# zengxianyu/sketchedit

Measured on NVIDIA H100. Metric: images/sec 256x256 CelebA-HQ generator fwd, higher is better.
Workload: dtype bf16

## Files before the change

sketchedit_b200/csrc/se_conv_c8.cu:

```cuda
#include "se_conv_c8.h"

#include <stdlib.h>

#include <map>
#include <mutex>

#include "se_tc_device.cuh"

namespace se {

constexpr int C8_TH = 16, C8_TW = 8;
constexpr int C8_CONSUMER_WARPS = 8;
constexpr int C8_THREADS = 32 * C8_CONSUMER_WARPS + 32;
constexpr int C8_MAX_STAGES = 8;

__device__ __forceinline__ void ring_of(int i, int n, int shift, int& slot, uint32_t& phase) {
  if (shift >= 0) { slot = i & (n - 1); phase = (uint32_t)(i >> shift) & 1u; }
  else { const int qd = i / n; slot = i - qd * n; phase = (uint32_t)qd & 1u; }
}

template <int NT, bool kF16, int R64, int M64, int R32>
__global__ void __launch_bounds__(C8_THREADS, 1)
conv_c8_kernel(const __grid_constant__ CUtensorMap tmA, const C8Params p) {
  extern __shared__ __align__(1024) uint8_t smem_raw[];
  uint8_t* smem = reinterpret_cast<uint8_t*>((reinterpret_cast<uintptr_t>(smem_raw) + 1023) & ~uintptr_t(1023));
  const bool halo = (p.mode == C8_HALO);
  constexpr int b64_bytes = NT * 128, b32_bytes = NT * 64;
  constexpr int b_bytes = R64 * b64_bytes + R32 * b32_bytes;
  const int stage_a = halo ? 0 : p.a_bytes;
  const int stage_b = p.resident ? 0 : b_bytes;
  const int stage_bytes = stage_a + stage_b;
  const bool staged = stage_bytes > 0;
  uint8_t* sHalo = smem;
  uint8_t* sWres = sHalo + (halo ? p.a_bufs * p.a_bytes : 0);
  uint8_t* sStages = sWres + (p.resident ? p.wres_bytes : 0);
  uint8_t* tail = sStages + (size_t)p.num_stages * stage_bytes;
  uint64_t* full_bar = reinterpret_cast<uint64_t*>(tail);
  uint64_t* empty_bar = full_bar + C8_MAX_STAGES;
  uint64_t* a_full = empty_bar + C8_MAX_STAGES;
  uint64_t* a_empty = a_full + C8_MAX_ABUFS;
  uint64_t* wres_bar = a_empty + C8_MAX_ABUFS;
  float* bias_s = reinterpret_cast<float*>(wres_bar + 2);

  const int warp = threadIdx.x >> 5;
  const int lane = threadIdx.x & 31;
  const bool clustered = p.cluster > 1;
  const uint32_t rank = clustered ? cluster_ctarank() : 0u;
  if (threadIdx.x == 0) {
    for (int i = 0; i < C8_MAX_STAGES; ++i) {
      mbar_init(&full_bar[i], 1);
      mbar_init(&empty_bar[i], C8_CONSUMER_WARPS * p.cluster);
    }
    for (int i = 0; i < C8_MAX_ABUFS; ++i) {
      mbar_init(&a_full[i], 1);
      mbar_init(&a_empty[i], C8_CONSUMER_WARPS);
    }
    mbar_init(wres_bar, 1);
    asm volatile("fence.mbarrier_init.release.cluster;" ::: "memory");
  }
  const int cst_n = NT + 32;
  epi_fill_constants(bias_s, cst_n, p.bias, p.e, threadIdx.x, C8_THREADS);
  if (clustered) cluster_sync();
  else __syncthreads();

  const int total_tiles = p.N * p.tiles_x * p.tiles_y;
  const int ksteps = p.ksteps;
  const int first_tile = (int)blockIdx.x - (int)rank;

  if (warp == C8_CONSUMER_WARPS) {
    if (lane == 0) asm volatile("prefetch.tensormap [%0];" ::"l"(reinterpret_cast<uint64_t>(&tmA)) : "memory");
    if (p.resident && elect_one()) {
      mbar_expect_tx(wres_bar, (uint32_t)p.wres_bytes);
      for (int off = 0; off < p.wres_bytes; off += 65536) {
        const int n = min(65536, p.wres_bytes - off);
        bulk_load_1d(sWres + off, p.w + off, (uint32_t)n, wres_bar);
      }
    }
    __syncwarp();
    const int b_split = (b_bytes >> 11) << 10;
    const int b_off = rank ? b_split : 0, b_len = clustered ? (rank ? b_bytes - b_split : b_split) : b_bytes;
    int stage = 0, iter = 0;
    uint32_t phase = 0;
    int tx = blockIdx.x % p.tiles_x, ty = (blockIdx.x / p.tiles_x) % p.tiles_y, img = blockIdx.x / (p.tiles_x * p.tiles_y);
    for (int tile = blockIdx.x; tile - (int)rank < total_tiles; tile += gridDim.x, ++iter) {
      if (tile != (int)blockIdx.x) {
        tx += p.step_x;
        if (tx >= p.tiles_x) { tx -= p.tiles_x; ++ty; }
        ty += p.step_y;
        if (ty >= p.tiles_y) { ty -= p.tiles_y; ++img; }
        img += p.step_img;
      }
      const int x0 = tx * C8_TW, y0 = ty * C8_TH;
      const bool load_a = tile < total_tiles;
      if (halo && load_a) {
        int ab;
        uint32_t aphase;
        ring_of(iter, p.a_bufs, p.a_shift, ab, aphase);
        mbar_wait(&a_empty[ab], aphase ^ 1, 5);
        if (elect_one()) {
          mbar_expect_tx(&a_full[ab], (uint32_t)p.a_tx_bytes);
          tma_load_4d(sHalo + (size_t)ab * p.a_bytes, &tmA, &a_full[ab], (x0 - p.pad_x0) * 8, y0 - p.pad_y0, p.x_cb_off, img);
        }
        __syncwarp();
      }
      if (staged) {
        for (int ks = 0; ks < ksteps; ++ks) {
          mbar_wait(&empty_bar[stage], phase ^ 1, 1);
          uint8_t* st = sStages + (size_t)stage * stage_bytes;
          if (elect_one()) {
            mbar_expect_tx(&full_bar[stage], (uint32_t)((halo || !load_a ? 0 : p.a_tx_bytes) + stage_b));
            if (!p.resident) {
              const uint8_t* src = p.w + (size_t)ks * b_bytes + b_off;
              if (clustered) bulk_load_1d_multicast(st + stage_a + b_off, src, (uint32_t)b_len, &full_bar[stage], 0x3);
              else bulk_load_1d(st + stage_a, src, (uint32_t)b_len, &full_bar[stage]);
            }
            if (!halo && load_a) {
              const int t = ks / p.cpt, ch = ks - t * p.cpt;
              tma_load_4d(st, &tmA, &full_bar[stage], (x0 + p.dx[t]) * 8, y0 + p.dy[t], p.x_cb_off + p.tap_cb[t] + 8 * ch, img);
            }
          }
          __syncwarp();
          if (++stage == p.num_stages) { stage = 0; phase ^= 1; }
        }
      }
    }
  } else {
    const int wg = warp >> 2, wq = warp & 3;
    const uint32_t smem_base = smem_u32(smem);
    const uint32_t off_wres = halo ? (uint32_t)(p.a_bufs * p.a_bytes) : 0u;
    const uint32_t off_stages = off_wres + (p.resident ? (uint32_t)p.wres_bytes : 0u);
    const uint32_t a_m = (uint32_t)wg * 8u * (uint32_t)p.sbo_bytes;
    const uint32_t n_u64 = p.ntaps * p.n64;
    const int ncls = p.ncls;
    const uint32_t tpi = (uint32_t)(p.tiles_x * p.tiles_y);
    const uint32_t cst_s = smem_u32(bias_s);
    const bool elu = p.e.epi == EPI_GATE_ELU, paired = p.e.paired != 0;
    if (p.resident) mbar_wait(wres_bar, 0, 6);
    auto release = [&](uint64_t* bar) {
      __syncwarp();
      if (lane == 0) mbar_arrive(bar);
    };
    auto release_stage = [&](int s) {
      __syncwarp();
      if (lane == 0) {
        mbar_arrive(&empty_bar[s]);
        if (clustered) mbar_arrive_cluster(&empty_bar[s], rank ^ 1u);
      }
    };
    float acc[NT / 2];
#pragma unroll
    for (int i = 0; i < NT / 2; ++i) acc[i] = 0.0f;
    int stage = 0;
    uint32_t phase = 0;
    const int my_tiles = (first_tile < total_tiles) ? (total_tiles - first_tile + (int)gridDim.x - 1) / (int)gridDim.x : 0;
    const int nv = my_tiles * ncls;
    const bool pingpong = p.resident && ksteps == 1;
    for (int v = 0; v < nv; ++v) {
      const int riter = ncls == 1 ? v : v / ncls, cls = v - riter * ncls;
      const int tile = (int)blockIdx.x + riter * (int)gridDim.x;
      if (tile >= total_tiles) {
        for (int ks = 0; ks < ksteps; ++ks) {
          mbar_wait(&full_bar[stage], phase, 3);
          release_stage(stage);
          if (++stage == p.num_stages) { stage = 0; phase ^= 1; }
        }
        continue;
      }
      const uint32_t img_u = (uint32_t)tile / tpi, rem = (uint32_t)tile - img_u * tpi;
      const uint32_t ty_u = rem / (uint32_t)p.tiles_x;
      const int img = (int)img_u, ty = (int)ty_u, tx = (int)(rem - ty_u * (uint32_t)p.tiles_x);
      int ab = 0;
      if (halo) {
        uint32_t aph;
        ring_of(riter, p.a_bufs, p.a_shift, ab, aph);
        mbar_wait(&a_full[ab], aph, 7);
      }
      if (pingpong && (wg == 1 || v > 0)) named_bar_sync(wg == 0 ? 2 : 1, 256);
      int prev = -1;
      for (int ks = 0; ks < ksteps; ++ks) {
        if (staged) mbar_wait(&full_bar[stage], phase, 3);
        const uint32_t st = smem_base + off_stages + (uint32_t)stage * stage_bytes;
        const uint32_t sB = p.resident ? smem_base + off_wres + (uint32_t)cls * (uint32_t)p.cls_bytes + (uint32_t)ks * b_bytes : st + stage_a;
        const uint32_t sA = (halo ? smem_base + (uint32_t)ab * p.a_bytes : st) + a_m;
        const int ub = cls * C8_CLS_UNITS;
        const int u0 = ub + ks * R64, v0 = ub + (int)n_u64 + ks * R32;
        const uint32_t acc0 = ks ? 1u : 0u;
        wg_fence();
        wg_fence_acc(acc);
#pragma unroll
        for (int j = 0; j < R64; ++j) {
          const uint32_t a0 = sA + p.aoff[u0 + j];
          const uint32_t b0 = sB + (uint32_t)(j * b64_bytes);
#pragma unroll
          for (int k = 0; k < M64; ++k)
            Wgmma<NT, kF16, 0>::mma(acc, wg_desc(a0 + k * p.kstep_bytes, p.lbo_bytes, p.sbo_bytes, WG_SW_NONE),
                                    wg_desc(b0 + 32u * k, 16u, 1024u, WG_SW128), j + k ? 1u : acc0);
        }
#pragma unroll
        for (int j = 0; j < R32; ++j) {
          const uint32_t a0 = sA + p.aoff[v0 + j];
          const uint32_t b0 = sB + (uint32_t)(R64 * b64_bytes + j * b32_bytes);
#pragma unroll
          for (int k = 0; k < 2; ++k)
            Wgmma<NT, kF16, 0>::mma(acc, wg_desc(a0 + k * p.kstep_bytes, p.lbo_bytes, p.sbo_bytes, WG_SW_NONE),
                                    wg_desc(b0 + 32u * k, 16u, 512u, WG_SW64), R64 + j + k ? 1u : acc0);
        }
        wg_commit();
        if (staged) {
          if (prev >= 0) {
            wg_wait<1>();
            release_stage(prev);
          }
          prev = stage;
          if (++stage == p.num_stages) { stage = 0; phase ^= 1; }
        }
      }
      if (pingpong && (wg == 0 || v + 1 < nv)) named_bar_arrive(wg == 0 ? 1 : 2, 256);
      wg_wait<0>();
      wg_fence_acc(acc);
      if (prev >= 0) release_stage(prev);
      if (halo && cls == ncls - 1) release(&a_empty[ab]);
      const int ooy = ncls > 1 ? p.cls_ooy[cls] : p.e.ooy, oox = ncls > 1 ? p.cls_oox[cls] : p.e.oox;
      size_t base[2];
      bool ok[2];
#pragma unroll
      for (int h = 0; h < 2; ++h) {
        const int ry = 8 * wg + 2 * wq + h, rx = lane >> 2;
        const int py = ty * C8_TH + ry, px = tx * C8_TW + rx;
        ok[h] = py < p.Ho && px < p.Wo;
        base[h] = epi_pixel_offset(p.e, img, py * p.e.osy + ooy, px * p.e.osx + oox, 2 * (lane & 3));
      }
      if (elu) {
        if (kF16 || paired) conv_epilogue<NT, kF16, true, true>(p.e, cst_s, acc, base, ok, lane);
        else conv_epilogue<NT, false, true, false>(p.e, cst_s, acc, base, ok, lane);
      } else {
        if (kF16 || paired) conv_epilogue<NT, kF16, false, true>(p.e, cst_s, acc, base, ok, lane);
        else conv_epilogue<NT, false, false, false>(p.e, cst_s, acc, base, ok, lane);
      }
    }
  }
  if (clustered) cluster_sync();
}

void fill_epi(const ConvParams& c, int NT, EpiParams* e) {
  e->y = c.y; e->out_c8 = c.out_c8;
  e->Hout = c.Hout; e->Wout = c.Wout; e->ldo = c.ldo; e->choff = c.choff;
  e->osy = c.osy; e->ooy = c.ooy; e->osx = c.osx; e->oox = c.oox;
  e->epi = c.epi; e->scale = c.scale;
  e->Cout = c.Cout; e->NT = NT;
  e->blk_split = c.out_blk_split > 0 ? c.out_blk_split : (1 << 20);
  e->blk_jump = c.out_blk_split > 0 ? c.out_blk_jump : 0;
  e->par_stride = c.out_par_stride > 0 ? c.out_par_stride : (c.ldo >> 2);
  const long long plane = c.out_c8 == 2 ? (long long)(c.Hout / 2) * (c.Wout / 2) : (long long)c.Hout * c.Wout;
  e->blk_stride = (int)(c.out_c8 ? plane * 8 : 8);
  e->goff = gated_goff(c.Cout);
  e->paired = (c.out_c8 != 0 || (((c.ldo | c.choff) & 1) == 0 && c.Cout / 2 == e->goff)) ? 1 : 0;
  e->split_stride = (int)c.out_split_stride;
}
typedef CUresult (*EncodeTiledFn)(CUtensorMap*, CUtensorMapDataType, cuuint32_t, void*, const cuuint64_t*, const cuuint64_t*,
                                  const cuuint32_t*, const cuuint32_t*, CUtensorMapInterleave, CUtensorMapSwizzle,
                                  CUtensorMapL2promotion, CUtensorMapFloatOOBfill);
static EncodeTiledFn c8_encode_fn() {
  static EncodeTiledFn fn = nullptr;
  if (!fn) {
    void* p = nullptr;
    cudaDriverEntryPointQueryResult qres;
    if (cudaGetDriverEntryPoint("cuTensorMapEncodeTiled", &p, cudaEnableDefault, &qres) != cudaSuccess || qres != cudaDriverEntryPointSuccess || !p) return nullptr;
    fn = reinterpret_cast<EncodeTiledFn>(p);
  }
  return fn;
// ... 36 lines not shown
  L->mode = (halo_bytes <= 72 * 1024) ? C8_HALO : C8_PERTAP;
  if (L->mode == C8_HALO) {
    L->HR = HR; L->WR = WR; L->pad_y0 = -mn_y; L->pad_x0 = -mn_x;
  } else {
    L->HR = C8_TH; L->WR = C8_TW; L->pad_y0 = 0; L->pad_x0 = 0;
    L->cb_in = (w.n64 * 64 + w.n32 * 32) / 8;
  }
  L->a_tx_bytes = L->cb_in * L->HR * L->WR * 16;
  L->a_bytes = (L->a_tx_bytes + 1023) / 1024 * 1024;
  L->resident = (wbytes <= kResidentMax) && (2 * L->a_bytes + wbytes <= kSmemBudget);
  if (L->resident && L->mode == C8_HALO) {
    w.r64 = ntaps * w.n64;
    w.r32 = ntaps * w.n32;
  } else if (L->mode == C8_PERTAP || (w.n64 > 0 && w.n32 > 0)) { w.r64 = w.n64; w.r32 = w.n32; }
  else {
    const int unit = w.n64 ? w.NT * 128 : w.NT * 64, total = ntaps * (w.n64 ? w.n64 : w.n32);
    int best = 1;
    for (int k = 1; k <= 8 && k <= total; ++k)
      if (total % k == 0 && k * unit <= 48 * 1024) best = k;
    if (w.n64) { w.r64 = best; w.r32 = 0; } else { w.r64 = 0; w.r32 = best; }
  }
  if (L->mode == C8_PERTAP && w.n32 == 0 && w.n64 > 1 && 2 * (L->a_bytes + w.NT * w.n64 * 128) > kSmemBudget) {
    L->chunks_per_tap = w.n64;
    L->cb_in = 8;
    L->a_tx_bytes = L->cb_in * L->HR * L->WR * 16;
    L->a_bytes = (L->a_tx_bytes + 1023) / 1024 * 1024;
    w.r64 = 1;
  }
  if (L->mode == C8_PERTAP) SE_REQUIRE(tc_ksteps(w) == ntaps * L->chunks_per_tap, "per-tap stages must be whole taps or whole chunks");
  return 0;
}

typedef void (*C8Kernel)(CUtensorMap, C8Params);
struct C8Inst { int nt; bool f16; int r64, m64, r32; C8Kernel fn; };
#define C8_INST(nt, f16, r64, m64, r32) {nt, f16, r64, m64, r32, conv_c8_kernel<nt, f16, r64, m64, r32>}
static const C8Inst kC8Insts[] = {
    C8_INST(32, false, 0, 0, 9),
    C8_INST(48, false, 0, 0, 9),
    C8_INST(48, false, 4, 3, 0),
    C8_INST(48, false, 5, 3, 0),
    C8_INST(96, false, 0, 0, 9),
    C8_INST(96, false, 4, 4, 4),
    C8_INST(96, false, 5, 3, 0),
    C8_INST(96, false, 9, 3, 0),
    C8_INST(96, false, 3, 3, 0),
    C8_INST(192, false, 1, 3, 0),
    C8_INST(192, false, 1, 4, 0),
    C8_INST(192, false, 1, 4, 1),
    C8_INST(32, true, 0, 0, 27),
    C8_INST(48, true, 0, 0, 3),
    C8_INST(48, true, 12, 3, 0),
    C8_INST(48, true, 15, 3, 0),
    C8_INST(96, true, 0, 0, 3),
    C8_INST(96, true, 1, 3, 0),
    C8_INST(96, true, 1, 4, 1),
    C8_INST(96, true, 3, 3, 0),
    C8_INST(192, true, 1, 3, 0),
    C8_INST(192, true, 1, 4, 0),
    C8_INST(192, true, 1, 4, 1),
};
#undef C8_INST
static C8Kernel c8_kernel(const C8Layer& L, bool f16) {
  const TcWeights& w = L.w;
  const int r64 = w.n64 ? w.r64 : 0, r32 = w.n32 ? w.r32 : 0, m64 = r64 ? L.mmas64 : 0;
  for (const C8Inst& k : kC8Insts)
    if (k.nt == w.NT && k.f16 == f16 && k.r64 == r64 && k.m64 == m64 && k.r32 == r32) return k.fn;
  return nullptr;
}
static int c8_set_smem_attr(int bytes) {
  for (const C8Inst& k : kC8Insts) SE_CUDA_OK(cudaFuncSetAttribute(k.fn, cudaFuncAttributeMaxDynamicSharedMemorySize, bytes));
  return 0;
}
int c8_instantiated(const C8Layer& L, bool f16, const std::string& name) {
  const TcWeights& w = L.w;
  SE_REQUIRE(c8_kernel(L, f16) != nullptr,
             "layer " + name + (f16 ? " (split-half)" : "") + ": no conv_c8_kernel instantiation for N = " + std::to_string(w.NT) +
                 ", k-step of " + std::to_string(w.n64 ? w.r64 : 0) + " x " + std::to_string(L.mmas64) + " + " +
                 std::to_string(w.n32 ? w.r32 : 0) + " x 2 MMAs (se_conv_c8.cu: kC8Insts)");
  return 0;
}
static void c8_launch_config(cudaLaunchConfig_t* cfg, cudaLaunchAttribute* attr, int grid, int smem_bytes, int cluster, cudaStream_t stream) {
  *cfg = cudaLaunchConfig_t();
  cfg->gridDim = dim3(grid);
  cfg->blockDim = dim3(C8_THREADS);
  cfg->dynamicSmemBytes = smem_bytes;
  cfg->stream = stream;
  if (cluster > 1) {
    attr->id = cudaLaunchAttributeClusterDimension;
    attr->val.clusterDim.x = cluster;
    attr->val.clusterDim.y = 1;
    attr->val.clusterDim.z = 1;
    cfg->attrs = attr;
    cfg->numAttrs = 1;
  }
}
static int c8_max_clusters(C8Kernel k, int smem_bytes, int* out) {
  static std::mutex mu;
  static std::map<std::pair<C8Kernel, int>, int> cache;
  std::lock_guard<std::mutex> lock(mu);
  auto it = cache.find({k, smem_bytes});
  if (it == cache.end()) {
    cudaLaunchConfig_t cfg;
    cudaLaunchAttribute attr;
    c8_launch_config(&cfg, &attr, 2 * g_sms, smem_bytes, 2, 0);
    int n = 0;
    SE_CUDA_OK(cudaOccupancyMaxActiveClusters(&n, k, &cfg));
    SE_REQUIRE(n > 0, "no 2-CTA cluster of conv_c8_kernel fits on the device");
    it = cache.emplace(std::make_pair(k, smem_bytes), n).first;
  }
  *out = it->second;
  return 0;
}

static const int kGroupSmemMax = 222 * 1024;

int c8_configure_group(C8Group* G, int ncls, int ntaps, const int8_t (*dy)[8], const int8_t (*dx)[8], const int* ooy, const int* oox, int Ci, int Cout) {
  if (ncls < 2 || ncls > C8_MAX_CLS || ntaps > 8) return 1;
  int mn_y = 0, mx_y = 0, mn_x = 0, mx_x = 0;
  for (int c = 0; c < ncls; ++c)
    for (int t = 0; t < ntaps; ++t) {
      mn_y = dy[c][t] < mn_y ? dy[c][t] : mn_y; mx_y = dy[c][t] > mx_y ? dy[c][t] : mx_y;
      mn_x = dx[c][t] < mn_x ? dx[c][t] : mn_x; mx_x = dx[c][t] > mx_x ? dx[c][t] : mx_x;
    }
  C8Layer& L = G->geo;
  L = C8Layer();
  TcWeights& w = L.w;
  w.ntaps = ntaps;
  w.n64 = Ci / 64;
  int rem = Ci - 64 * w.n64;
  if (rem > 32) { ++w.n64; rem = 0; }
  w.n32 = rem > 0 ? 1 : 0;
  w.NT = (gated_goff(Cout) + Cout / 2 + 15) / 16 * 16;
  w.n_tiles = 1;
  w.img_bytes = 0;
  w.r64 = ntaps * w.n64;
  w.r32 = ntaps * w.n32;
  L.mmas64 = Ci == 48 ? 3 : 4;
// ... 51 lines not shown
  p.cls_bytes = grp ? grp->cls_bytes : 0;
  for (int k = 0; k < C8_MAX_CLS; ++k) { p.cls_ooy[k] = grp && k < grp->ncls ? grp->ooy[k] : 0; p.cls_oox[k] = grp && k < grp->ncls ? grp->oox[k] : 0; }
  if (L.stem) { p.lbo_bytes = 16; p.kstep_bytes = 32; }
  else { p.lbo_bytes = L.HR * L.WR * 16; p.kstep_bytes = 2 * p.lbo_bytes; }
  p.sbo_bytes = L.WR * 16;
  p.bias = c.bias;
  fill_epi(c, w.NT, &p.e);
  {
    const bool halo = (L.mode == C8_HALO);
    const int n_u64 = c.ntaps * w.n64, n_u32 = c.ntaps * w.n32;
    SE_REQUIRE(n_u64 + n_u32 < C8_MAX_UNITS, "too many K units");
    SE_REQUIRE(!grp || n_u64 + n_u32 <= C8_CLS_UNITS, "too many K units per class");
    for (int k = 0; k < (grp ? grp->ncls : 1); ++k)
      for (int u = 0; u < n_u64 + n_u32; ++u) {
        const bool is64 = u < n_u64;
        const int t = is64 ? u / w.n64 : u - n_u64;
        const int cb0 = L.chunks_per_tap > 1 ? 0 : (halo ? L.tap_cb[t] : 0) + (is64 ? (u - t * w.n64) * 8 : w.n64 * 8);
        const int tdy = grp ? grp->dy[k][t] : c.dy[t], tdx = grp ? grp->dx[k][t] : c.dx[t];
        const int oy = halo ? tdy + L.pad_y0 : 0, ox = halo ? tdx + L.pad_x0 : 0;
        p.aoff[k * C8_CLS_UNITS + u] = (uint32_t)((cb0 * L.HR + oy) * L.WR + ox) * 16u;
      }
  }
  SE_REQUIRE(c.Cout % 2 == 0 && (c.out_dt == DT_BF16 || c.out_dt == DT_F16X2), "gated epilogue needs even Cout, 16-bit out");
  SE_REQUIRE(!c.out_c8 || c.choff % 8 == 0, "C8 output needs a channel offset multiple of 8");
  SE_REQUIRE(!c.f16x2 || c.out_c8 != 0, "split-half output is channel-blocked");
  SE_REQUIRE(c.out_c8 != 2 || (c.Hout % 2 == 0 && c.Wout % 2 == 0 && c.ldo % 4 == 0 && (c.Cout / 2) % 8 == 0),
             "space-to-depth output: even size, whole channel blocks");
  {
    const long long plane = c.out_c8 == 2 ? (long long)(c.Hout / 2) * (c.Wout / 2) : (long long)c.Hout * c.Wout;
    SE_REQUIRE((long long)(w.NT / 16) * (c.out_c8 ? 8 * plane : 8) + 8LL * p.e.blk_jump < (1LL << 31), "output block offsets must fit in 31 bits");
  }

  const int total_tiles = p.N * p.tiles_x * p.tiles_y;
  const int smem_budget = grp ? kGroupSmemMax - 4096 : kSmemBudget;
  const int b_bytes = tc_stage_b_bytes(w);
  const int stage_bytes = (L.mode == C8_HALO ? 0 : L.a_bytes) + (L.resident ? 0 : b_bytes);
  int fixed = (L.resident ? p.wres_bytes : 0);
  p.a_bufs = 2;
  if (L.mode == C8_HALO) {
    if (fixed + 2 * L.a_bytes + 3 * stage_bytes > smem_budget) p.a_bufs = 1;
    if (stage_bytes == 0)
      while (p.a_bufs < C8_MAX_ABUFS && fixed + 2 * p.a_bufs * L.a_bytes <= smem_budget) p.a_bufs *= 2;
    fixed += p.a_bufs * L.a_bytes;
  }
  p.a_shift = -1;
  for (int sh = 0; sh < 4; ++sh) if ((1 << sh) == p.a_bufs) p.a_shift = sh;
  SE_REQUIRE(p.a_bufs <= C8_MAX_ABUFS, "halo ring plan");
  SE_REQUIRE(!grp || (p.a_bufs >= 2 && p.ksteps == 1), "fused classes need two halo buffers and a single k-step");
  SE_REQUIRE(!(L.resident && p.ksteps == 1) || p.a_bufs >= 2, "ping-pong warpgroups need two halo buffers");
  int stages = stage_bytes ? (smem_budget - fixed) / stage_bytes : 1;
  if (stages > C8_MAX_STAGES) stages = C8_MAX_STAGES;
  SE_REQUIRE(stages >= (stage_bytes ? 2 : 1), "shared memory plan does not fit");
  p.num_stages = stages;
  const int smem_bytes = 1024 + fixed + stages * stage_bytes + (2 * C8_MAX_STAGES + 2 * C8_MAX_ABUFS + 2) * 8 + 3 * (p.NT + 32) * 4 + 64;

  EncodeTiledFn enc = c8_encode_fn();
  SE_REQUIRE(enc != nullptr, "cuTensorMapEncodeTiled not available from the driver");
  if (!g_sms) {
    int dev = 0;
    SE_CUDA_OK(cudaGetDevice(&dev));
    SE_CUDA_OK(cudaDeviceGetAttribute(&g_sms, cudaDevAttrMultiProcessorCount, dev));
    SE_CUDA_OK(cudaDeviceGetAttribute(&g_optin, cudaDevAttrMaxSharedMemoryPerBlockOptin, dev));
    { int rc_attr = c8_set_smem_attr(g_optin); if (rc_attr) return rc_attr; }
  }
  SE_REQUIRE(smem_bytes <= g_optin, "shared memory plan exceeds the opt-in limit");

  CUtensorMap tmA;
  {
    cuuint64_t dims[4] = {(cuuint64_t)c.Wi * 8, (cuuint64_t)c.Hi, (cuuint64_t)c.ldx, (cuuint64_t)c.N};
    cuuint64_t strides[3] = {(cuuint64_t)c.Wi * 16, (cuuint64_t)c.Hi * c.Wi * 16, (cuuint64_t)c.ldx * c.Hi * c.Wi * 16};
    cuuint32_t box[4] = {(cuuint32_t)(L.WR * 8), (cuuint32_t)L.HR, (cuuint32_t)L.cb_in, 1};
    cuuint32_t estr[4] = {1, 1, 1, 1};
    CUresult r = enc(&tmA, CU_TENSOR_MAP_DATA_TYPE_BFLOAT16, 4, const_cast<void*>(c.x), dims, strides, box, estr,
                     CU_TENSOR_MAP_INTERLEAVE_NONE, CU_TENSOR_MAP_SWIZZLE_NONE, CU_TENSOR_MAP_L2_PROMOTION_L2_256B,
                     CU_TENSOR_MAP_FLOAT_OOB_FILL_NONE);
    SE_REQUIRE(r == CUDA_SUCCESS, "cuTensorMapEncodeTiled(C8) failed, CUresult=" + std::to_string((int)r));
  }
  const C8Kernel kernel = c8_kernel(L, p.f16 != 0);
  SE_REQUIRE(kernel != nullptr, "no conv_c8_kernel instantiation for the layer's plan (N = " + std::to_string(p.NT) + ")");
  p.cluster = L.resident ? 1 : 2;
  int grid = total_tiles < g_sms ? total_tiles : g_sms;
  if (p.cluster > 1) {
    int max_clusters = 0;
    { int rc_occ = c8_max_clusters(kernel, smem_bytes, &max_clusters); if (rc_occ) return rc_occ; }
    const int pairs = (total_tiles + 1) / 2;
    grid = 2 * (pairs < max_clusters ? pairs : max_clusters);
  }
  p.step_x = grid % p.tiles_x;
  p.step_y = (grid / p.tiles_x) % p.tiles_y;
  p.step_img = grid / (p.tiles_x * p.tiles_y);
  cudaLaunchConfig_t cfg;
  cudaLaunchAttribute attr;
  c8_launch_config(&cfg, &attr, grid, smem_bytes, p.cluster, stream);
  SE_CUDA_OK(cudaLaunchKernelEx(&cfg, kernel, tmA, p));
  return 0;
}

}
```

sketchedit_b200/csrc/se_tc_device.cuh:

```cuda
#pragma once
#include <cuda_fp16.h>

#include "se_common.cuh"
#include "se_wgmma.cuh"

namespace se {

__device__ __forceinline__ uint32_t smem_u32(const void* p) { return (uint32_t)__cvta_generic_to_shared(p); }

__device__ __forceinline__ void mbar_init(uint64_t* bar, uint32_t count) {
  asm volatile("mbarrier.init.shared::cta.b64 [%0], %1;" ::"r"(smem_u32(bar)), "r"(count));
}
__device__ __forceinline__ void mbar_expect_tx(uint64_t* bar, uint32_t bytes) {
  asm volatile("mbarrier.arrive.expect_tx.shared::cta.b64 _, [%0], %1;" ::"r"(smem_u32(bar)), "r"(bytes) : "memory");
}
__device__ __forceinline__ void mbar_arrive(uint64_t* bar) {
  asm volatile("mbarrier.arrive.shared::cta.b64 _, [%0];" ::"r"(smem_u32(bar)) : "memory");
}
__device__ __forceinline__ void mbar_wait(uint64_t* bar, uint32_t parity, int tag) {
  (void)tag;
  asm volatile(
      "{\n\t.reg .pred p;\n\t.reg .b64 t0, t1;\n\t.reg .b32 n;\n\t"
      "mov.u64 t0, 0;\n\t"
      "OUTER_%=:\n\t"
// ... 32 lines not shown
               : "memory");
}

__device__ __forceinline__ uint32_t cluster_ctarank() {
  uint32_t r;
  asm volatile("mov.u32 %0, %%cluster_ctarank;" : "=r"(r));
  return r;
}
__device__ __forceinline__ void cluster_sync() {
  asm volatile("barrier.cluster.arrive.release;\n\tbarrier.cluster.wait.acquire;" ::: "memory");
}
__device__ __forceinline__ void mbar_arrive_cluster(uint64_t* bar, uint32_t cta) {
  asm volatile("{\n\t.reg .b32 ra;\n\tmapa.shared::cluster.u32 ra, %0, %1;\n\tmbarrier.arrive.release.cta.shared::cluster.b64 _, [ra];\n\t}"
               ::"r"(smem_u32(bar)), "r"(cta) : "memory");
}

__device__ __forceinline__ bool elect_one() {
  uint32_t pred;
  asm volatile("{\n\t.reg .pred p;\n\telect.sync _|p, 0xffffffff;\n\tselp.u32 %0, 1, 0, p;\n\t}" : "=r"(pred));
  return pred != 0;
}

enum : uint32_t { WG_SW_NONE = 0, WG_SW128 = 1, WG_SW64 = 2 };
__device__ __forceinline__ uint64_t wg_desc(uint32_t smem_addr, uint32_t lbo_bytes, uint32_t sbo_bytes, uint32_t layout) {
  return (uint64_t)((smem_addr & 0x3FFFF) >> 4) | ((uint64_t)((lbo_bytes >> 4) & 0x3FFF) << 16) |
         ((uint64_t)((sbo_bytes >> 4) & 0x3FFF) << 32) | ((uint64_t)layout << 62);
}
__device__ __forceinline__ void wg_fence() { asm volatile("wgmma.fence.sync.aligned;" ::: "memory"); }
__device__ __forceinline__ void wg_commit() { asm volatile("wgmma.commit_group.sync.aligned;" ::: "memory"); }
template <int N>
__device__ __forceinline__ void wg_wait() { asm volatile("wgmma.wait_group.sync.aligned %0;" ::"n"(N) : "memory"); }
__device__ __forceinline__ void named_bar_sync(int id, int n) { asm volatile("bar.sync %0, %1;" ::"r"(id), "r"(n) : "memory"); }
__device__ __forceinline__ void named_bar_arrive(int id, int n) { asm volatile("bar.arrive %0, %1;" ::"r"(id), "r"(n) : "memory"); }
template <int R>
__device__ __forceinline__ void wg_fence_acc(float (&d)[R]) {
#pragma unroll
  for (int i = 0; i < R; ++i) asm volatile("" : "+f"(d[i])::"memory");
}
__device__ __forceinline__ int frag_row(int w, int lane, int h) { return 16 * w + (lane >> 2) + 8 * h; }
__device__ __forceinline__ int frag_col(int lane, int j) { return 8 * j + 2 * (lane & 3); }

__device__ __forceinline__ float tanh_approx(float x) {
  float y;
  asm("tanh.approx.f32 %0, %1;" : "=f"(y) : "f"(x));
  return y;
}
__device__ __forceinline__ float ex2_approx(float x) {
  float y;
  asm("ex2.approx.ftz.f32 %0, %1;" : "=f"(y) : "f"(x));
  return y;
}
__device__ __forceinline__ float rcp_approx(float x) {
  float y;
  asm("rcp.approx.ftz.f32 %0, %1;" : "=f"(y) : "f"(x));
  return y;
}
__device__ __forceinline__ uint32_t pack_f16x2(float lo, float hi) {
  __half2 v = __floats2half2_rn(lo, hi);
  return *reinterpret_cast<uint32_t*>(&v);
}

__device__ __forceinline__ void epi_fill_constants(float* cst, int n, const float* bias, const EpiParams& e, int tid, int nthreads) {
  const int half = e.Cout >> 1;
  for (int i = tid; i < n; i += nthreads) {
    const int ch = i < half ? i : (i >= e.goff && i < e.goff + half ? half + i - e.goff : -1);
    const float b = (bias != nullptr && ch >= 0 && ch < e.Cout) ? bias[ch] : 0.0f;
// ... 104 lines not shown
```

Baseline: 4725.

## Add ping-pong consumer warpgroups with full-tile accumulators for streamed-weight convs

Adds a ping-pong variant of the implicit-GEMM conv kernel. Each consumer warpgroup now owns a whole 16-row tile with two accumulator sets and alternates tiles with the other warpgroup through named barriers, so one group's epilogue overlaps the other's WGMMA mainloop. The variant adds a full producer warpgroup and uses setmaxnreg to move registers to the consumers. It is selected for non-resident, non-f16 layers with at least two tiles per SM, and it raises the shared-memory budget for those layers. The cost is higher register pressure, fewer pipeline stages per stage reader, and a more complex launch path.

```diff
diff --git a/sketchedit_b200/csrc/se_conv_c8.cu b/sketchedit_b200/csrc/se_conv_c8.cu
--- a/sketchedit_b200/csrc/se_conv_c8.cu
+++ b/sketchedit_b200/csrc/se_conv_c8.cu
@@ -12,6 +12,8 @@
 constexpr int C8_TH = 16, C8_TW = 8;
 constexpr int C8_CONSUMER_WARPS = 8;
 constexpr int C8_THREADS = 32 * C8_CONSUMER_WARPS + 32;
+constexpr int C8_PP_THREADS = 32 * C8_CONSUMER_WARPS + 128;
+constexpr int C8_PP_PRODUCER_REGS = 40, C8_PP_CONSUMER_REGS = 232;
 constexpr int C8_MAX_STAGES = 8;
 
 __device__ __forceinline__ void ring_of(int i, int n, int shift, int& slot, uint32_t& phase) {
@@ -19,9 +21,11 @@
   else { const int qd = i / n; slot = i - qd * n; phase = (uint32_t)qd & 1u; }
 }
 
-template <int NT, bool kF16, int R64, int M64, int R32>
-__global__ void __launch_bounds__(C8_THREADS, 1)
+template <int NT, bool kF16, int R64, int M64, int R32, bool kPP>
+__global__ void __launch_bounds__(kPP ? C8_PP_THREADS : C8_THREADS, 1)
 conv_c8_kernel(const __grid_constant__ CUtensorMap tmA, const C8Params p) {
+  constexpr int kThreads = kPP ? C8_PP_THREADS : C8_THREADS;
+  constexpr int kStageReaders = kPP ? 4 : C8_CONSUMER_WARPS;
   extern __shared__ __align__(1024) uint8_t smem_raw[];
   uint8_t* smem = reinterpret_cast<uint8_t*>((reinterpret_cast<uintptr_t>(smem_raw) + 1023) & ~uintptr_t(1023));
   const bool halo = (p.mode == C8_HALO);
@@ -49,17 +53,17 @@
   if (threadIdx.x == 0) {
     for (int i = 0; i < C8_MAX_STAGES; ++i) {
       mbar_init(&full_bar[i], 1);
-      mbar_init(&empty_bar[i], C8_CONSUMER_WARPS * p.cluster);
+      mbar_init(&empty_bar[i], kStageReaders * p.cluster);
     }
     for (int i = 0; i < C8_MAX_ABUFS; ++i) {
       mbar_init(&a_full[i], 1);
-      mbar_init(&a_empty[i], C8_CONSUMER_WARPS);
+      mbar_init(&a_empty[i], kStageReaders);
     }
     mbar_init(wres_bar, 1);
     asm volatile("fence.mbarrier_init.release.cluster;" ::: "memory");
   }
   const int cst_n = NT + 32;
-  epi_fill_constants(bias_s, cst_n, p.bias, p.e, threadIdx.x, C8_THREADS);
+  epi_fill_constants(bias_s, cst_n, p.bias, p.e, threadIdx.x, kThreads);
   if (clustered) cluster_sync();
   else __syncthreads();
 
@@ -67,69 +71,72 @@
   const int ksteps = p.ksteps;
   const int first_tile = (int)blockIdx.x - (int)rank;
 
-  if (warp == C8_CONSUMER_WARPS) {
-    if (lane == 0) asm volatile("prefetch.tensormap [%0];" ::"l"(reinterpret_cast<uint64_t>(&tmA)) : "memory");
-    if (p.resident && elect_one()) {
-      mbar_expect_tx(wres_bar, (uint32_t)p.wres_bytes);
-      for (int off = 0; off < p.wres_bytes; off += 65536) {
-        const int n = min(65536, p.wres_bytes - off);
-        bulk_load_1d(sWres + off, p.w + off, (uint32_t)n, wres_bar);
-      }
-    }
-    __syncwarp();
-    const int b_split = (b_bytes >> 11) << 10;
-    const int b_off = rank ? b_split : 0, b_len = clustered ? (rank ? b_bytes - b_split : b_split) : b_bytes;
-    int stage = 0, iter = 0;
-    uint32_t phase = 0;
-    int tx = blockIdx.x % p.tiles_x, ty = (blockIdx.x / p.tiles_x) % p.tiles_y, img = blockIdx.x / (p.tiles_x * p.tiles_y);
-    for (int tile = blockIdx.x; tile - (int)rank < total_tiles; tile += gridDim.x, ++iter) {
-      if (tile != (int)blockIdx.x) {
-        tx += p.step_x;
-        if (tx >= p.tiles_x) { tx -= p.tiles_x; ++ty; }
-        ty += p.step_y;
-        if (ty >= p.tiles_y) { ty -= p.tiles_y; ++img; }
-        img += p.step_img;
-      }
-      const int x0 = tx * C8_TW, y0 = ty * C8_TH;
-      const bool load_a = tile < total_tiles;
-      if (halo && load_a) {
-        int ab;
-        uint32_t aphase;
-        ring_of(iter, p.a_bufs, p.a_shift, ab, aphase);
-        mbar_wait(&a_empty[ab], aphase ^ 1, 5);
-        if (elect_one()) {
-          mbar_expect_tx(&a_full[ab], (uint32_t)p.a_tx_bytes);
-          tma_load_4d(sHalo + (size_t)ab * p.a_bytes, &tmA, &a_full[ab], (x0 - p.pad_x0) * 8, y0 - p.pad_y0, p.x_cb_off, img);
-        }
-        __syncwarp();
-      }
-      if (staged) {
-        for (int ks = 0; ks < ksteps; ++ks) {
-          mbar_wait(&empty_bar[stage], phase ^ 1, 1);
-          uint8_t* st = sStages + (size_t)stage * stage_bytes;
+  if (warp >= C8_CONSUMER_WARPS) {
+    if constexpr (kPP) setmaxnreg_dec<C8_PP_PRODUCER_REGS>();
+    if (warp == C8_CONSUMER_WARPS) {
+      if (lane == 0) asm volatile("prefetch.tensormap [%0];" ::"l"(reinterpret_cast<uint64_t>(&tmA)) : "memory");
+      if (p.resident && elect_one()) {
+        mbar_expect_tx(wres_bar, (uint32_t)p.wres_bytes);
+        for (int off = 0; off < p.wres_bytes; off += 65536) {
+          const int n = min(65536, p.wres_bytes - off);
+          bulk_load_1d(sWres + off, p.w + off, (uint32_t)n, wres_bar);
+        }
+      }
+      __syncwarp();
+      const int b_split = (b_bytes >> 11) << 10;
+      const int b_off = rank ? b_split : 0, b_len = clustered ? (rank ? b_bytes - b_split : b_split) : b_bytes;
+      int stage = 0, iter = 0;
+      uint32_t phase = 0;
+      int tx = blockIdx.x % p.tiles_x, ty = (blockIdx.x / p.tiles_x) % p.tiles_y, img = blockIdx.x / (p.tiles_x * p.tiles_y);
+      for (int tile = blockIdx.x; tile - (int)rank < total_tiles; tile += gridDim.x, ++iter) {
+        if (tile != (int)blockIdx.x) {
+          tx += p.step_x;
+          if (tx >= p.tiles_x) { tx -= p.tiles_x; ++ty; }
+          ty += p.step_y;
+          if (ty >= p.tiles_y) { ty -= p.tiles_y; ++img; }
+          img += p.step_img;
+        }
+        const int x0 = tx * C8_TW, y0 = ty * C8_TH;
+        const bool load_a = tile < total_tiles;
+        if (halo && load_a) {
+          int ab;
+          uint32_t aphase;
+          ring_of(iter, p.a_bufs, p.a_shift, ab, aphase);
+          mbar_wait(&a_empty[ab], aphase ^ 1, 5);
           if (elect_one()) {
-            mbar_expect_tx(&full_bar[stage], (uint32_t)((halo || !load_a ? 0 : p.a_tx_bytes) + stage_b));
-            if (!p.resident) {
-              const uint8_t* src = p.w + (size_t)ks * b_bytes + b_off;
-              if (clustered) bulk_load_1d_multicast(st + stage_a + b_off, src, (uint32_t)b_len, &full_bar[stage], 0x3);
-              else bulk_load_1d(st + stage_a, src, (uint32_t)b_len, &full_bar[stage]);
-            }
-            if (!halo && load_a) {
-              const int t = ks / p.cpt, ch = ks - t * p.cpt;
-              tma_load_4d(st, &tmA, &full_bar[stage], (x0 + p.dx[t]) * 8, y0 + p.dy[t], p.x_cb_off + p.tap_cb[t] + 8 * ch, img);
-            }
+            mbar_expect_tx(&a_full[ab], (uint32_t)p.a_tx_bytes);
+            tma_load_4d(sHalo + (size_t)ab * p.a_bytes, &tmA, &a_full[ab], (x0 - p.pad_x0) * 8, y0 - p.pad_y0, p.x_cb_off, img);
           }
           __syncwarp();
-          if (++stage == p.num_stages) { stage = 0; phase ^= 1; }
+        }
+        if (staged) {
+          for (int ks = 0; ks < ksteps; ++ks) {
+            mbar_wait(&empty_bar[stage], phase ^ 1, 1);
+            uint8_t* st = sStages + (size_t)stage * stage_bytes;
+            if (elect_one()) {
+              mbar_expect_tx(&full_bar[stage], (uint32_t)((halo || !load_a ? 0 : p.a_tx_bytes) + stage_b));
+              if (!p.resident) {
+                const uint8_t* src = p.w + (size_t)ks * b_bytes + b_off;
+                if (clustered) bulk_load_1d_multicast(st + stage_a + b_off, src, (uint32_t)b_len, &full_bar[stage], 0x3);
+                else bulk_load_1d(st + stage_a, src, (uint32_t)b_len, &full_bar[stage]);
+              }
+              if (!halo && load_a) {
+                const int t = ks / p.cpt, ch = ks - t * p.cpt;
+                tma_load_4d(st, &tmA, &full_bar[stage], (x0 + p.dx[t]) * 8, y0 + p.dy[t], p.x_cb_off + p.tap_cb[t] + 8 * ch, img);
+              }
+            }
+            __syncwarp();
+            if (++stage == p.num_stages) { stage = 0; phase ^= 1; }
+          }
         }
       }
     }
   } else {
+    if constexpr (kPP) setmaxnreg_inc<C8_PP_CONSUMER_REGS>();
     const int wg = warp >> 2, wq = warp & 3;
     const uint32_t smem_base = smem_u32(smem);
     const uint32_t off_wres = halo ? (uint32_t)(p.a_bufs * p.a_bytes) : 0u;
     const uint32_t off_stages = off_wres + (p.resident ? (uint32_t)p.wres_bytes : 0u);
-    const uint32_t a_m = (uint32_t)wg * 8u * (uint32_t)p.sbo_bytes;
     const uint32_t n_u64 = p.ntaps * p.n64;
     const int ncls = p.ncls;
     const uint32_t tpi = (uint32_t)(p.tiles_x * p.tiles_y);
@@ -147,66 +154,87 @@
         if (clustered) mbar_arrive_cluster(&empty_bar[s], rank ^ 1u);
       }
     };
-    float acc[NT / 2];
+    auto issue_kstep = [&](float (&a)[NT / 2], uint32_t sA, uint32_t sB, int u0, int v0, uint32_t acc0) {
 #pragma unroll
-    for (int i = 0; i < NT / 2; ++i) acc[i] = 0.0f;
-    int stage = 0;
-    uint32_t phase = 0;
+      for (int j = 0; j < R64; ++j) {
+        const uint32_t a0 = sA + p.aoff[u0 + j];
+        const uint32_t b0 = sB + (uint32_t)(j * b64_bytes);
+#pragma unroll
+        for (int k = 0; k < M64; ++k)
+          Wgmma<NT, kF16, 0>::mma(a, wg_desc(a0 + k * p.kstep_bytes, p.lbo_bytes, p.sbo_bytes, WG_SW_NONE),
+                                  wg_desc(b0 + 32u * k, 16u, 1024u, WG_SW128), j + k ? 1u : acc0);
+      }
+#pragma unroll
+      for (int j = 0; j < R32; ++j) {
+        const uint32_t a0 = sA + p.aoff[v0 + j];
+        const uint32_t b0 = sB + (uint32_t)(R64 * b64_bytes + j * b32_bytes);
+#pragma unroll
+        for (int k = 0; k < 2; ++k)
+          Wgmma<NT, kF16, 0>::mma(a, wg_desc(a0 + k * p.kstep_bytes, p.lbo_bytes, p.sbo_bytes, WG_SW_NONE),
+                                  wg_desc(b0 + 32u * k, 16u, 512u, WG_SW64), R64 + j + k ? 1u : acc0);
+      }
+    };
+    auto epilogue = [&](const float (&a)[NT / 2], int row8, int img, int ty, int tx, int cls) {
+      const int ooy = ncls > 1 ? p.cls_ooy[cls] : p.e.ooy, oox = ncls > 1 ? p.cls_oox[cls] : p.e.oox;
+      size_t base[2];
+      bool ok[2];
+#pragma unroll
+      for (int h = 0; h < 2; ++h) {
+        const int ry = row8 + 2 * wq + h, rx = lane >> 2;
+        const int py = ty * C8_TH + ry, px = tx * C8_TW + rx;
+        ok[h] = py < p.Ho && px < p.Wo;
+        base[h] = epi_pixel_offset(p.e, img, py * p.e.osy + ooy, px * p.e.osx + oox, 2 * (lane & 3));
+      }
+      if (elu) {
+        if (kF16 || paired) conv_epilogue<NT, kF16, true, true>(p.e, cst_s, a, base, ok, lane);
+        else conv_epilogue<NT, false, true, false>(p.e, cst_s, a, base, ok, lane);
+      } else {
+        if (kF16 || paired) conv_epilogue<NT, kF16, false, true>(p.e, cst_s, a, base, ok, lane);
+        else conv_epilogue<NT, false, false, false>(p.e, cst_s, a, base, ok, lane);
+      }
+    };
     const int my_tiles = (first_tile < total_tiles) ? (total_tiles - first_tile + (int)gridDim.x - 1) / (int)gridDim.x : 0;
-    const int nv = my_tiles * ncls;
-    const bool pingpong = p.resident && ksteps == 1;
-    for (int v = 0; v < nv; ++v) {
-      const int riter = ncls == 1 ? v : v / ncls, cls = v - riter * ncls;
-      const int tile = (int)blockIdx.x + riter * (int)gridDim.x;
-      if (tile >= total_tiles) {
+    if constexpr (kPP) {
+      float acc[2][NT / 2];
+#pragma unroll
+      for (int i = 0; i < NT / 2; ++i) acc[0][i] = acc[1][i] = 0.0f;
+      for (int riter = wg; riter < my_tiles; riter += 2) {
+        const int tile = (int)blockIdx.x + riter * (int)gridDim.x;
+        int stage;
+        uint32_t phase;
+        ring_of(riter * ksteps, p.num_stages, -1, stage, phase);
+        if (riter > 0) named_bar_sync(wg == 0 ? 2 : 1, 256);
+        if (tile >= total_tiles) {
+          for (int ks = 0; ks < ksteps; ++ks) {
+            mbar_wait(&full_bar[stage], phase, 3);
+            release_stage(stage);
+            if (++stage == p.num_stages) { stage = 0; phase ^= 1; }
+          }
+          continue;
+        }
+        const uint32_t img_u = (uint32_t)tile / tpi, rem = (uint32_t)tile - img_u * tpi;
+        const uint32_t ty_u = rem / (uint32_t)p.tiles_x;
+        const int img = (int)img_u, ty = (int)ty_u, tx = (int)(rem - ty_u * (uint32_t)p.tiles_x);
+        int ab = 0;
+        if (halo) {
+          uint32_t aph;
+          ring_of(riter, p.a_bufs, p.a_shift, ab, aph);
+          mbar_wait(&a_full[ab], aph, 7);
+        }
+        const uint32_t a_hi = 8u * (uint32_t)p.sbo_bytes;
+        int prev = -1;
         for (int ks = 0; ks < ksteps; ++ks) {
           mbar_wait(&full_bar[stage], phase, 3);
-          release_stage(stage);
-          if (++stage == p.num_stages) { stage = 0; phase ^= 1; }
-        }
-        continue;
-      }
-      const uint32_t img_u = (uint32_t)tile / tpi, rem = (uint32_t)tile - img_u * tpi;
-      const uint32_t ty_u = rem / (uint32_t)p.tiles_x;
-      const int img = (int)img_u, ty = (int)ty_u, tx = (int)(rem - ty_u * (uint32_t)p.tiles_x);
-      int ab = 0;
-      if (halo) {
-        uint32_t aph;
-        ring_of(riter, p.a_bufs, p.a_shift, ab, aph);
-        mbar_wait(&a_full[ab], aph, 7);
-      }
-      if (pingpong && (wg == 1 || v > 0)) named_bar_sync(wg == 0 ? 2 : 1, 256);
-      int prev = -1;
-      for (int ks = 0; ks < ksteps; ++ks) {
-        if (staged) mbar_wait(&full_bar[stage], phase, 3);
-        const uint32_t st = smem_base + off_stages + (uint32_t)stage * stage_bytes;
-        const uint32_t sB = p.resident ? smem_base + off_wres + (uint32_t)cls * (uint32_t)p.cls_bytes + (uint32_t)ks * b_bytes : st + stage_a;
-        const uint32_t sA = (halo ? smem_base + (uint32_t)ab * p.a_bytes : st) + a_m;
-        const int ub = cls * C8_CLS_UNITS;
-        const int u0 = ub + ks * R64, v0 = ub + (int)n_u64 + ks * R32;
-        const uint32_t acc0 = ks ? 1u : 0u;
-        wg_fence();
-        wg_fence_acc(acc);
-#pragma unroll
-        for (int j = 0; j < R64; ++j) {
-          const uint32_t a0 = sA + p.aoff[u0 + j];
-          const uint32_t b0 = sB + (uint32_t)(j * b64_bytes);
-#pragma unroll
-          for (int k = 0; k < M64; ++k)
-            Wgmma<NT, kF16, 0>::mma(acc, wg_desc(a0 + k * p.kstep_bytes, p.lbo_bytes, p.sbo_bytes, WG_SW_NONE),
-                                    wg_desc(b0 + 32u * k, 16u, 1024u, WG_SW128), j + k ? 1u : acc0);
-        }
-#pragma unroll
-        for (int j = 0; j < R32; ++j) {
-          const uint32_t a0 = sA + p.aoff[v0 + j];
-          const uint32_t b0 = sB + (uint32_t)(R64 * b64_bytes + j * b32_bytes);
-#pragma unroll
-          for (int k = 0; k < 2; ++k)
-            Wgmma<NT, kF16, 0>::mma(acc, wg_desc(a0 + k * p.kstep_bytes, p.lbo_bytes, p.sbo_bytes, WG_SW_NONE),
-                                    wg_desc(b0 + 32u * k, 16u, 512u, WG_SW64), R64 + j + k ? 1u : acc0);
-        }
-        wg_commit();
-        if (staged) {
+          const uint32_t st = smem_base + off_stages + (uint32_t)stage * stage_bytes;
+          const uint32_t sA = halo ? smem_base + (uint32_t)ab * p.a_bytes : st;
+          const int u0 = ks * R64, v0 = (int)n_u64 + ks * R32;
+          const uint32_t acc0 = ks ? 1u : 0u;
+          wg_fence();
+          wg_fence_acc(acc[0]);
+          wg_fence_acc(acc[1]);
+          issue_kstep(acc[0], sA, st + stage_a, u0, v0, acc0);
+          issue_kstep(acc[1], sA + a_hi, st + stage_a, u0, v0, acc0);
+          wg_commit();
           if (prev >= 0) {
             wg_wait<1>();
             release_stage(prev);
@@ -214,28 +242,71 @@
           prev = stage;
           if (++stage == p.num_stages) { stage = 0; phase ^= 1; }
         }
-      }
-      if (pingpong && (wg == 0 || v + 1 < nv)) named_bar_arrive(wg == 0 ? 1 : 2, 256);
-      wg_wait<0>();
-      wg_fence_acc(acc);
-      if (prev >= 0) release_stage(prev);
-      if (halo && cls == ncls - 1) release(&a_empty[ab]);
-      const int ooy = ncls > 1 ? p.cls_ooy[cls] : p.e.ooy, oox = ncls > 1 ? p.cls_oox[cls] : p.e.oox;
-      size_t base[2];
-      bool ok[2];
+        if (riter + 1 < my_tiles) named_bar_arrive(wg == 0 ? 1 : 2, 256);
+        wg_wait<0>();
+        wg_fence_acc(acc[0]);
+        wg_fence_acc(acc[1]);
+        release_stage(prev);
+        if (halo) release(&a_empty[ab]);
+        epilogue(acc[0], 0, img, ty, tx, 0);
+        epilogue(acc[1], 8, img, ty, tx, 0);
+      }
+    } else {
+      float acc[NT / 2];
 #pragma unroll
-      for (int h = 0; h < 2; ++h) {
-        const int ry = 8 * wg + 2 * wq + h, rx = lane >> 2;
-        const int py = ty * C8_TH + ry, px = tx * C8_TW + rx;
-        ok[h] = py < p.Ho && px < p.Wo;
-        base[h] = epi_pixel_offset(p.e, img, py * p.e.osy + ooy, px * p.e.osx + oox, 2 * (lane & 3));
-      }
-      if (elu) {
-        if (kF16 || paired) conv_epilogue<NT, kF16, true, true>(p.e, cst_s, acc, base, ok, lane);
-        else conv_epilogue<NT, false, true, false>(p.e, cst_s, acc, base, ok, lane);
-      } else {
-        if (kF16 || paired) conv_epilogue<NT, kF16, false, true>(p.e, cst_s, acc, base, ok, lane);
-        else conv_epilogue<NT, false, false, false>(p.e, cst_s, acc, base, ok, lane);
+      for (int i = 0; i < NT / 2; ++i) acc[i] = 0.0f;
+      int stage = 0;
+      uint32_t phase = 0;
+      const int nv = my_tiles * ncls;
+      const bool pingpong = p.resident && ksteps == 1;
+      const uint32_t a_m = (uint32_t)wg * 8u * (uint32_t)p.sbo_bytes;
+      for (int v = 0; v < nv; ++v) {
+        const int riter = ncls == 1 ? v : v / ncls, cls = v - riter * ncls;
+        const int tile = (int)blockIdx.x + riter * (int)gridDim.x;
+        if (tile >= total_tiles) {
+          for (int ks = 0; ks < ksteps; ++ks) {
+            mbar_wait(&full_bar[stage], phase, 3);
+            release_stage(stage);
+            if (++stage == p.num_stages) { stage = 0; phase ^= 1; }
+          }
+          continue;
+        }
+        const uint32_t img_u = (uint32_t)tile / tpi, rem = (uint32_t)tile - img_u * tpi;
+        const uint32_t ty_u = rem / (uint32_t)p.tiles_x;
+        const int img = (int)img_u, ty = (int)ty_u, tx = (int)(rem - ty_u * (uint32_t)p.tiles_x);
+        int ab = 0;
+        if (halo) {
+          uint32_t aph;
+          ring_of(riter, p.a_bufs, p.a_shift, ab, aph);
+          mbar_wait(&a_full[ab], aph, 7);
+        }
+        if (pingpong && (wg == 1 || v > 0)) named_bar_sync(wg == 0 ? 2 : 1, 256);
+        int prev = -1;
+        for (int ks = 0; ks < ksteps; ++ks) {
+          if (staged) mbar_wait(&full_bar[stage], phase, 3);
+          const uint32_t st = smem_base + off_stages + (uint32_t)stage * stage_bytes;
+          const uint32_t sB = p.resident ? smem_base + off_wres + (uint32_t)cls * (uint32_t)p.cls_bytes + (uint32_t)ks * b_bytes : st + stage_a;
+          const uint32_t sA = (halo ? smem_base + (uint32_t)ab * p.a_bytes : st) + a_m;
+          const int ub = cls * C8_CLS_UNITS;
+          wg_fence();
+          wg_fence_acc(acc);
+          issue_kstep(acc, sA, sB, ub + ks * R64, ub + (int)n_u64 + ks * R32, ks ? 1u : 0u);
+          wg_commit();
+          if (staged) {
+            if (prev >= 0) {
+              wg_wait<1>();
+              release_stage(prev);
+            }
+            prev = stage;
+            if (++stage == p.num_stages) { stage = 0; phase ^= 1; }
+          }
+        }
+        if (pingpong && (wg == 0 || v + 1 < nv)) named_bar_arrive(wg == 0 ? 1 : 2, 256);
+        wg_wait<0>();
+        wg_fence_acc(acc);
+        if (prev >= 0) release_stage(prev);
+        if (halo && cls == ncls - 1) release(&a_empty[ab]);
+        epilogue(acc, 8 * wg, img, ty, tx, cls);
       }
     }
   }
@@ -338,8 +409,9 @@
 }
 
 typedef void (*C8Kernel)(CUtensorMap, C8Params);
-struct C8Inst { int nt; bool f16; int r64, m64, r32; C8Kernel fn; };
-#define C8_INST(nt, f16, r64, m64, r32) {nt, f16, r64, m64, r32, conv_c8_kernel<nt, f16, r64, m64, r32>}
+struct C8Inst { int nt; bool f16; int r64, m64, r32; bool pp; C8Kernel fn; };
+#define C8_INST(nt, f16, r64, m64, r32) {nt, f16, r64, m64, r32, false, conv_c8_kernel<nt, f16, r64, m64, r32, false>}
+#define C8_INST_PP(nt, r64, m64, r32) {nt, false, r64, m64, r32, true, conv_c8_kernel<nt, false, r64, m64, r32, true>}
 static const C8Inst kC8Insts[] = {
     C8_INST(32, false, 0, 0, 9),
     C8_INST(48, false, 0, 0, 9),
@@ -349,6 +421,10 @@
     C8_INST(96, false, 4, 4, 4),
     C8_INST(96, false, 5, 3, 0),
     C8_INST(96, false, 9, 3, 0),
+    C8_INST_PP(96, 3, 3, 0),
+    C8_INST_PP(192, 1, 3, 0),
+    C8_INST_PP(192, 1, 4, 0),
+    C8_INST_PP(192, 1, 4, 1),
     C8_INST(96, false, 3, 3, 0),
     C8_INST(192, false, 1, 3, 0),
     C8_INST(192, false, 1, 4, 0),
@@ -366,11 +442,13 @@
     C8_INST(192, true, 1, 4, 1),
 };
 #undef C8_INST
-static C8Kernel c8_kernel(const C8Layer& L, bool f16) {
+#undef C8_INST_PP
+static bool c8_pingpong_tiles(const C8Layer& L, bool f16, long long tiles, int sms) { return !L.resident && !f16 && tiles >= 2LL * sms; }
+static C8Kernel c8_kernel(const C8Layer& L, bool f16, bool pp) {
   const TcWeights& w = L.w;
   const int r64 = w.n64 ? w.r64 : 0, r32 = w.n32 ? w.r32 : 0, m64 = r64 ? L.mmas64 : 0;
   for (const C8Inst& k : kC8Insts)
-    if (k.nt == w.NT && k.f16 == f16 && k.r64 == r64 && k.m64 == m64 && k.r32 == r32) return k.fn;
+    if (k.nt == w.NT && k.f16 == f16 && k.r64 == r64 && k.m64 == m64 && k.r32 == r32 && k.pp == pp) return k.fn;
   return nullptr;
 }
 static int c8_set_smem_attr(int bytes) {
@@ -379,16 +457,17 @@
 }
 int c8_instantiated(const C8Layer& L, bool f16, const std::string& name) {
   const TcWeights& w = L.w;
-  SE_REQUIRE(c8_kernel(L, f16) != nullptr,
+  SE_REQUIRE(c8_kernel(L, f16, false) != nullptr && (L.resident || f16 || c8_kernel(L, f16, true) != nullptr),
              "layer " + name + (f16 ? " (split-half)" : "") + ": no conv_c8_kernel instantiation for N = " + std::to_string(w.NT) +
                  ", k-step of " + std::to_string(w.n64 ? w.r64 : 0) + " x " + std::to_string(L.mmas64) + " + " +
                  std::to_string(w.n32 ? w.r32 : 0) + " x 2 MMAs (se_conv_c8.cu: kC8Insts)");
   return 0;
 }
-static void c8_launch_config(cudaLaunchConfig_t* cfg, cudaLaunchAttribute* attr, int grid, int smem_bytes, int cluster, cudaStream_t stream) {
+static void c8_launch_config(cudaLaunchConfig_t* cfg, cudaLaunchAttribute* attr, int grid, int threads, int smem_bytes, int cluster,
+                             cudaStream_t stream) {
   *cfg = cudaLaunchConfig_t();
   cfg->gridDim = dim3(grid);
-  cfg->blockDim = dim3(C8_THREADS);
+  cfg->blockDim = dim3(threads);
   cfg->dynamicSmemBytes = smem_bytes;
   cfg->stream = stream;
   if (cluster > 1) {
@@ -400,7 +479,7 @@
     cfg->numAttrs = 1;
   }
 }
-static int c8_max_clusters(C8Kernel k, int smem_bytes, int* out) {
+static int c8_max_clusters(C8Kernel k, int threads, int smem_bytes, int* out) {
   static std::mutex mu;
   static std::map<std::pair<C8Kernel, int>, int> cache;
   std::lock_guard<std::mutex> lock(mu);
@@ -408,7 +487,7 @@
   if (it == cache.end()) {
     cudaLaunchConfig_t cfg;
     cudaLaunchAttribute attr;
-    c8_launch_config(&cfg, &attr, 2 * g_sms, smem_bytes, 2, 0);
+    c8_launch_config(&cfg, &attr, 2 * g_sms, threads, smem_bytes, 2, 0);
     int n = 0;
     SE_CUDA_OK(cudaOccupancyMaxActiveClusters(&n, k, &cfg));
     SE_REQUIRE(n > 0, "no 2-CTA cluster of conv_c8_kernel fits on the device");
@@ -526,7 +605,15 @@
   }
 
   const int total_tiles = p.N * p.tiles_x * p.tiles_y;
-  const int smem_budget = grp ? kGroupSmemMax - 4096 : kSmemBudget;
+  if (!g_sms) {
+    int dev = 0;
+    SE_CUDA_OK(cudaGetDevice(&dev));
+    SE_CUDA_OK(cudaDeviceGetAttribute(&g_sms, cudaDevAttrMultiProcessorCount, dev));
+    SE_CUDA_OK(cudaDeviceGetAttribute(&g_optin, cudaDevAttrMaxSharedMemoryPerBlockOptin, dev));
+    { int rc_attr = c8_set_smem_attr(g_optin); if (rc_attr) return rc_attr; }
+  }
+  const bool pp = c8_pingpong_tiles(L, c.f16x2 != 0, total_tiles, g_sms);
+  const int smem_budget = grp || pp ? kGroupSmemMax - 4096 : kSmemBudget;
   const int b_bytes = tc_stage_b_bytes(w);
   const int stage_bytes = (L.mode == C8_HALO ? 0 : L.a_bytes) + (L.resident ? 0 : b_bytes);
   int fixed = (L.resident ? p.wres_bytes : 0);
@@ -550,13 +637,6 @@
 
   EncodeTiledFn enc = c8_encode_fn();
   SE_REQUIRE(enc != nullptr, "cuTensorMapEncodeTiled not available from the driver");
-  if (!g_sms) {
-    int dev = 0;
-    SE_CUDA_OK(cudaGetDevice(&dev));
-    SE_CUDA_OK(cudaDeviceGetAttribute(&g_sms, cudaDevAttrMultiProcessorCount, dev));
-    SE_CUDA_OK(cudaDeviceGetAttribute(&g_optin, cudaDevAttrMaxSharedMemoryPerBlockOptin, dev));
-    { int rc_attr = c8_set_smem_attr(g_optin); if (rc_attr) return rc_attr; }
-  }
   SE_REQUIRE(smem_bytes <= g_optin, "shared memory plan exceeds the opt-in limit");
 
   CUtensorMap tmA;
@@ -570,13 +650,14 @@
                      CU_TENSOR_MAP_FLOAT_OOB_FILL_NONE);
     SE_REQUIRE(r == CUDA_SUCCESS, "cuTensorMapEncodeTiled(C8) failed, CUresult=" + std::to_string((int)r));
   }
-  const C8Kernel kernel = c8_kernel(L, p.f16 != 0);
+  const C8Kernel kernel = c8_kernel(L, p.f16 != 0, pp);
+  const int threads = pp ? C8_PP_THREADS : C8_THREADS;
   SE_REQUIRE(kernel != nullptr, "no conv_c8_kernel instantiation for the layer's plan (N = " + std::to_string(p.NT) + ")");
   p.cluster = L.resident ? 1 : 2;
   int grid = total_tiles < g_sms ? total_tiles : g_sms;
   if (p.cluster > 1) {
     int max_clusters = 0;
-    { int rc_occ = c8_max_clusters(kernel, smem_bytes, &max_clusters); if (rc_occ) return rc_occ; }
+    { int rc_occ = c8_max_clusters(kernel, threads, smem_bytes, &max_clusters); if (rc_occ) return rc_occ; }
     const int pairs = (total_tiles + 1) / 2;
     grid = 2 * (pairs < max_clusters ? pairs : max_clusters);
   }
@@ -585,7 +666,7 @@
   p.step_img = grid / (p.tiles_x * p.tiles_y);
   cudaLaunchConfig_t cfg;
   cudaLaunchAttribute attr;
-  c8_launch_config(&cfg, &attr, grid, smem_bytes, p.cluster, stream);
+  c8_launch_config(&cfg, &attr, grid, threads, smem_bytes, p.cluster, stream);
   SE_CUDA_OK(cudaLaunchKernelEx(&cfg, kernel, tmA, p));
   return 0;
 }
diff --git a/sketchedit_b200/csrc/se_tc_device.cuh b/sketchedit_b200/csrc/se_tc_device.cuh
--- a/sketchedit_b200/csrc/se_tc_device.cuh
+++ b/sketchedit_b200/csrc/se_tc_device.cuh
@@ -88,6 +88,10 @@
 __device__ __forceinline__ void wg_wait() { asm volatile("wgmma.wait_group.sync.aligned %0;" ::"n"(N) : "memory"); }
 __device__ __forceinline__ void named_bar_sync(int id, int n) { asm volatile("bar.sync %0, %1;" ::"r"(id), "r"(n) : "memory"); }
 __device__ __forceinline__ void named_bar_arrive(int id, int n) { asm volatile("bar.arrive %0, %1;" ::"r"(id), "r"(n) : "memory"); }
+template <int N>
+__device__ __forceinline__ void setmaxnreg_inc() { asm volatile("setmaxnreg.inc.sync.aligned.u32 %0;" ::"n"(N)); }
+template <int N>
+__device__ __forceinline__ void setmaxnreg_dec() { asm volatile("setmaxnreg.dec.sync.aligned.u32 %0;" ::"n"(N)); }
 template <int R>
 __device__ __forceinline__ void wg_fence_acc(float (&d)[R]) {
 #pragma unroll
```

After: 4878, median of 6. 1.03x the previous value.
